# mvrl/RANGE

Hardware: AMD Instinct MI355X
Metric: geo-embeddings/sec (10k-query batch, range_db_large) (higher is better)
Workload: dtype f32

## Files before the change

### range_amd/csrc/engine_ctx.h

```cpp
#pragma once

struct Switches {
    bool allow_keep = true;
    bool enc_split = true;
    bool enc_fused = true;
    bool topks_force_exact = false;
    bool topks_bf16 = true;
    bool topks_fused = true;
    bool small_forward = true;
    bool topk_gemm = true;
    int tg_sample = TG_SAMPLE;
    bool p2_streamk = true;
};

static Switches parse_switches() {
    Switches sw;
    if (const char* e = std::getenv("RANGE_KEEP_LOGITS")) sw.allow_keep = e[0] != '0';
    if (const char* e = std::getenv("RANGE_ENC_SPLIT")) sw.enc_split = e[0] != '0';
    if (const char* e = std::getenv("RANGE_ENC_FUSED")) sw.enc_fused = e[0] != '0';
    if (const char* e = std::getenv("RANGE_TOPKS_FORCE_EXACT")) sw.topks_force_exact = e[0] == '1';
    if (const char* e = std::getenv("RANGE_TOPKS_KEYS")) sw.topks_bf16 = std::strcmp(e, "f32") != 0;
    if (const char* e = std::getenv("RANGE_TOPKS_FUSED")) sw.topks_fused = e[0] != '0';
    if (const char* e = std::getenv("RANGE_SMALL_FORWARD")) sw.small_forward = e[0] != '0';
    if (const char* e = std::getenv("RANGE_TOPK_GEMM")) sw.topk_gemm = e[0] != '0';
    if (const char* e = std::getenv("RANGE_TG_SAMPLE")) sw.tg_sample = std::max(1, std::min(16, std::atoi(e)));
    if (const char* e = std::getenv("RANGE_P2_STREAMK")) sw.p2_streamk = e[0] != '0';
    return sw;
}

struct range_ctx {
    int device = 0;
    int n_cu = 256;
    Switches sw;
    struct Encoder {
        bool has_encoder = false;
        range_encoder_desc desc{};
        EncArgs args{};
        size_t lds_bytes = 0;
        size_t lds_base = 0;
        DevBuf<int32_t> d_slot_base;
        DevBuf<double> d_coefA, d_coefB, d_seedc;
        DevBuf<double> d_wp[ENC_MAX_LAYERS], d_bias[ENC_MAX_LAYERS];
        DevBuf<SHDesc> d_sh_desc;
        DevBuf<double> d_sh_coef;
        DevBuf<int32_t> d_sh_pow;
        DevBuf<double> ws_h1, ws_h1a, ws_h2, ws_e3;
        DevBuf<uint32_t> ws_enc_sync;
    } enc;
    struct Bank {
        bool has_bank = false;
        bool has_values = false;
        int64_t n_rows = 0, n_pad = 0, row_offset = 0;
        DevBuf<float> d_keys, d_values, d_xyz4;
        DevBuf<uint32_t> d_keys_bf16;
        DevBuf<uint32_t> d_keys_f16;
        float tg_key_scale = 0.f;
        float key_norm_max = 1.f;
        float xyz_norm_max = 1.f;
        int pv_mode = RANGE_PV_EXACT;
        DevBuf<uint32_t> d_vplanes;
        int64_t vplanes_groups = 0;
    } bank;
    float tau_sem_set = 0.f, tau_geo_set = 0.f;
    struct Passes {
        DevBuf<double> ws_ehat64;
        DevBuf<float> ws_ehat32, ws_xq, ws_stats;
        int64_t ws_queries = 0;
        DevBuf<float> ws_stats_parts, ws_slabs;
        DevBuf<float> ws_small_o, ws_small_z;
        int last_qtiles = 0, last_splits = 0;
    } pass;
    struct Kept {
        DevBuf<float> ws_logits, ws_rowmax, ws_theta;
        DevBuf<float> ws_stat_parts;
        int64_t kept_B = 0, kept_total = 0;
        int32_t kept_blocks = 0;
        bool warned_no_keep = false;
    } kept;
    struct Topk {
// ... 2 lines not shown
        DevBuf<unsigned long long> ws_cand_keys;
        DevBuf<float> ws_cand_dmax;
        DevBuf<int32_t> ws_exact_count;
        DevBuf<uint32_t> ws_topk_sync;
        uint32_t topk_sync_base[8] = {0, 0, 0, 0, 0, 0, 0, 0};
        DevBuf<float> ws_tg_gmax, ws_tg_theta;
        DevBuf<uint32_t> ws_tg_qfrag;
        DevBuf<float> ws_tg_qscale;
        DevBuf<uint32_t> ws_tg_cnt, ws_tg_ovf;
        DevBuf<uint2> ws_tg_cand;
        DevBuf<uint32_t> ws_read_sink;
    } topk;
    struct Posenc {
        struct Table { std::vector<double> host; DevBuf<double> dev; };
        std::vector<std::unique_ptr<Table>> tables;
    } posenc;
    struct Csp {
        bool has = false;
        int kind = 0, F = 0, act = 0;
        bool skip = false, layn = false;
        int widths[CSP_MAX_LAYERS] = {};
        CspPlan plan;
        DevBuf<float> d_params;
        DevBuf<double> d_freq;
        DevBuf<CspLayerArgs> d_layers;
        int num_classes = 0;
        DevBuf<float> d_head;
        DevBuf<float> ws_feats;
        DevBuf<double> ws_rank;
    } csp;
    struct Checker {
        DevBuf<double> ws_a;
        DevBuf<int64_t> ws_idx;
    } checker;
    struct Neighbors {
        int64_t N = 0;
        int C = 0;
        bool hav = false, has_cells = false;
        DevBuf<NeighborPoint> d_pts;
        DevBuf<int32_t> ws_counts;
        DevBuf<double> ws_redk;
        DevBuf<int64_t> ws_jlast;
    } nb;
    uint32_t* h_async_err = nullptr;
    uint32_t* d_async_err = nullptr;
    bool debug_giveup_next = false;
    struct Host {
        DevBuf<double> ws_out64;
        void* h_stage = nullptr;
        size_t h_stage_bytes = 0;
        hipStream_t copy_stream = nullptr;
        std::unique_ptr<HostCopyPool> pool;
    } host;
    struct Profiling {
        bool on = false;
        std::vector<std::pair<hipEvent_t, hipEvent_t>> pairs[RANGE_PROF_KINDS];
    } prof;
    std::vector<hipEvent_t> ev_pool;
    hipEvent_t get_event() {
        if (!ev_pool.empty()) { hipEvent_t e = ev_pool.back(); ev_pool.pop_back(); return e; }
        hipEvent_t e = nullptr;
        (void)hipEventCreate(&e);
        return e;
    }
    ~range_ctx() {
        if (host.h_stage) (void)hipHostFree(host.h_stage);
        if (h_async_err) (void)hipHostFree(h_async_err);
        if (host.copy_stream) (void)hipStreamDestroy(host.copy_stream);
        for (auto& v : prof.pairs) for (auto& p : v) { (void)hipEventDestroy(p.first); (void)hipEventDestroy(p.second); }
        for (auto e : ev_pool) (void)hipEventDestroy(e);
    }
};

namespace {
struct ProfScope {
    range_ctx* c; int which; hipStream_t s; hipEvent_t a = nullptr, b = nullptr;
    ProfScope(range_ctx* c_, int which_, hipStream_t s_) : c(c_), which(which_), s(s_) {
        if (c->prof.on) { a = c->get_event(); b = c->get_event(); if (a) (void)hipEventRecord(a, s); }
    }
    ~ProfScope() {
        if (a && b) { (void)hipEventRecord(b, s); c->prof.pairs[which].emplace_back(a, b); }
    }
};

constexpr PlanConsts PLAN_CONSTS{QTILE, BLK, VAL_DIM, MAX_TOPK, P1_WG_PER_CU, ENC_QTILE, TOPKS_WL,
                                 TG_QBLOCK, TG_WG_PER_CU, TG_CAP_L};

template <typename... P, typename... A>
int launch(void (*kernel)(P...), dim3 grid, dim3 block, size_t lds, hipStream_t s, const A&... args) {
    if (lds)
        HIP_TRY(hipFuncSetAttribute(reinterpret_cast<const void*>(kernel),
                                    hipFuncAttributeMaxDynamicSharedMemorySize, (int)lds));
    hipLaunchKernelGGL(kernel, grid, block, lds, s, args...);
    HIP_TRY(hipGetLastError());
    return RANGE_OK;
}

template <typename F>
int timed_repeat(range_ctx* c, hipStream_t s, int repeats, float* avg_us, F&& body) {
    hipEvent_t ev0 = nullptr, ev1 = nullptr;
    if (repeats > 1) {
        ev0 = c->get_event();
        ev1 = c->get_event();
        HIP_TRY(hipEventRecord(ev0, s));
    }
    for (int rep = 0; rep < std::max(1, repeats); ++rep)
        if (int rc = body()) return rc;
    if (repeats > 1) {
        HIP_TRY(hipEventRecord(ev1, s));
        HIP_TRY(hipEventSynchronize(ev1));
        float ms = 0.f;
        HIP_TRY(hipEventElapsedTime(&ms, ev0, ev1));
        if (avg_us) *avg_us = ms * 1e3f / (float)repeats;
        c->ev_pool.push_back(ev0);
        c->ev_pool.push_back(ev1);
    }
    return RANGE_OK;
}

}

// ... 15 lines not shown
```

### range_amd/csrc/forward_host.h

```cpp
#pragma once

struct ModelParams { float tau_sem, tau_geo, beta; };

static int model_params(const range_ctx* c, int32_t model, float beta, ModelParams& m) {
    if (model != RANGE_MODEL_RANGE && model != RANGE_MODEL_RANGE_PLUS)
        return fail(RANGE_ERR_INVALID, "unknown model %d", model);
    m.tau_sem = model == RANGE_MODEL_RANGE ? 15.0f : 12.0f;
    m.tau_geo = model == RANGE_MODEL_RANGE ? 0.0f : 40.0f;
    if (c->tau_sem_set > 0.f) m.tau_sem = c->tau_sem_set;
    if (c->tau_geo_set > 0.f && model == RANGE_MODEL_RANGE_PLUS) m.tau_geo = c->tau_geo_set;
    m.beta = model == RANGE_MODEL_RANGE ? 1.0f : beta;
    return RANGE_OK;
}

static int forward_head(const range_ctx* c, const double* lonlat, const double* out, int32_t model, float beta, ModelParams& m) {
    if (!c || !lonlat || !out) return fail(RANGE_ERR_INVALID, "null argument");
    return model_params(c, model, beta, m);
}

static int forward_small(range_ctx* c, int64_t B, const ModelParams& m, double* out, hipStream_t s) {
    SmallArgs a{};
    int rc = softmax_scales(c, B, m.tau_sem, m.tau_geo, RANGE_MAX_TAU, a.k_sem, a.k_geo);
    if (rc) return rc;
    const SmallPlan p = plan_forward_small(c->n_cu, c->bank.n_rows, B, PLAN_CONSTS);
    HIP_TRY(c->pass.ws_small_o.ensure(p.o_floats));
    HIP_TRY(c->pass.ws_small_z.ensure(p.z_floats));
    a.keys = c->bank.d_keys.p;
    a.xyz4 = c->bank.d_xyz4.p;
    a.values = c->bank.d_values.p;
    a.ehat = c->pass.ws_ehat32.p;
    a.xq = c->pass.ws_xq.p;
    a.osum = c->pass.ws_small_o.p;
    a.zsum = c->pass.ws_small_z.p;
    a.B = B;
    a.n_valid = c->bank.n_rows;
    a.n_blocks = p.n_blocks;
    const bool geo = m.tau_geo > 0.f;
    static void (*const small_kernels[2][2])(SmallArgs) = {{attend_small_kernel<true, 2>, attend_small_kernel<true, 1>},
                                                          {attend_small_kernel<false, 2>, attend_small_kernel<false, 1>}};
    {
        ProfScope ps(c, RANGE_PROF_ATTEND, s);
        if (int lrc = launch(small_kernels[!geo][p.nq == 1], dim3((unsigned)p.n_wg), dim3(256), as_lds_bytes(p.nq), s, a)) return lrc;
    }
    rc = launch(small_finalize_kernel, dim3((unsigned)B, 8), dim3(1024), 0, s, c->pass.ws_small_o.p, c->pass.ws_small_z.p,
                p.n_wg, p.qcap, geo ? 1 : 0, geo ? m.beta : 1.0f, c->pass.ws_ehat64.p, out);
    if (rc) return rc;
    c->pass.last_qtiles = 1;
    c->pass.last_splits = p.n_wg;
    return RANGE_OK;
}

static int scan_workspace(range_ctx* c, int64_t B, const ModelParams& m, bool* kept, range_stream_t stream) {
    const int rc = range_scan_stats(c, c->pass.ws_ehat32.p, c->pass.ws_xq.p, B, m.tau_sem, m.tau_geo, c->pass.ws_stats.p, 0,
                                    nullptr, nullptr, 1, stream);
    *kept = c->kept.kept_B == B;
    return rc;
}

static int attend_workspace(range_ctx* c, int64_t p0, int64_t p1, const ModelParams& m, bool kept, SlabMap* map,
                            range_stream_t stream) {
    return attend_impl(c, c->pass.ws_ehat32.p + p0 * 256, c->pass.ws_xq.p + p0 * 4, p1 - p0, m.tau_sem, m.tau_geo, m.beta,
                       c->pass.ws_stats.p + p0 * 4, nullptr, map, kept ? p0 : -1, stream);
}

extern "C" {

int range_forward(range_ctx* c, const double* lonlat, int64_t B, int32_t model, float beta,
                  double* out, range_stream_t stream) {
    ModelParams m;
    if (int rc = forward_head(c, lonlat, out, model, beta, m)) return rc;
    c->pass.ws_queries = 0;
    if (int rc = encode_to_workspace(c, lonlat, B, nullptr, stream)) return rc;
    if (plan_temperatures(m.tau_sem, m.tau_geo, B, c->sw.small_forward).one_pass) {
        c->pass.ws_queries = B;
        ENTER_DEVICE(c);
        return forward_small(c, B, m, out, (hipStream_t)stream);
    }
    bool kept = false;
    SlabMap map{};
    if (int rc = scan_workspace(c, B, m, &kept, stream)) return rc;
    if (int rc = attend_workspace(c, 0, B, m, kept, &map, stream)) return rc;
    c->pass.ws_queries = B;
    ENTER_DEVICE(c);
    HIP_TRY(launch_finalize(c->pass.ws_slabs.p, map, c->pass.ws_ehat64.p, B, 0, B, out, (hipStream_t)stream));
    return RANGE_OK;
}

int range_host_copy(range_ctx* c, void* dst, const void* src, size_t bytes) {
    if (!c || !dst || !src) return fail(RANGE_ERR_INVALID, "null argument");
    if (!c->host.pool) c->host.pool.reset(new HostCopyPool(HostCopyPool::default_threads()));
    c->host.pool->copy(dst, src, bytes);
    return RANGE_OK;
}

int range_forward_host(range_ctx* c, const double* lonlat, int64_t B, int32_t model, float beta,
                       double* out_host, range_stream_t stream) {
    ModelParams m;
    if (int rc0 = forward_head(c, lonlat, out_host, model, beta, m)) return rc0;
    if (B <= 0) return fail(RANGE_ERR_INVALID, "B must be > 0");
    ENTER_DEVICE(c);
    hipStream_t s = (hipStream_t)stream;
    const size_t row_bytes = (size_t)RANGE_OUT_DIM * sizeof(double);
    HIP_TRY(c->host.ws_out64.ensure((size_t)B * RANGE_OUT_DIM));
    if (c->host.h_stage_bytes < (size_t)B * row_bytes) {
        if (c->host.h_stage) (void)hipHostFree(c->host.h_stage);
        c->host.h_stage = nullptr;
        c->host.h_stage_bytes = 0;
        HIP_TRY(hipHostMalloc(&c->host.h_stage, (size_t)B * row_bytes, hipHostMallocDefault));
        c->host.h_stage_bytes = (size_t)B * row_bytes;
    }
    if (!c->host.copy_stream) HIP_TRY(hipStreamCreateWithFlags(&c->host.copy_stream, hipStreamNonBlocking));
    if (!c->host.pool) c->host.pool.reset(new HostCopyPool(HostCopyPool::default_threads()));

    c->pass.ws_queries = 0;
    int rc = encode_to_workspace(c, lonlat, B, nullptr, stream);
    if (rc) return rc;
    c->pass.ws_queries = B;
    if (plan_temperatures(m.tau_sem, m.tau_geo, B, c->sw.small_forward).one_pass) {
        rc = forward_small(c, B, m, c->host.ws_out64.p, s);
        if (rc) return rc;
        HIP_TRY(hipMemcpyAsync(c->host.h_stage, c->host.ws_out64.p, (size_t)B * row_bytes, hipMemcpyDeviceToHost, s));
        HIP_TRY(hipStreamSynchronize(s));
        if (int rc2 = check_async_error(c)) return rc2;
        std::memcpy(out_host, c->host.h_stage, (size_t)B * row_bytes);
        return RANGE_OK;
    }
    bool kept = false;
    rc = scan_workspace(c, B, m, &kept, stream);
    if (rc) return rc;
// ... 56 lines not shown
```

### range_amd/csrc/host_plan.h

```cpp
#pragma once
#include <algorithm>
#include <cmath>
#include <cstddef>
#include <cstdint>
#include <vector>

namespace range_host {

inline int choose_splits(int n_qtiles, int n_blocks, int n_cu, int wg_per_cu, int max_splits,
                         double split_cost = 0.002) {
    const double slots = (double)n_cu * wg_per_cu;
    const int cap = std::max(1, std::min(max_splits, n_blocks / 4));
    const int ns_min = std::min(cap, (int)std::ceil(slots / n_qtiles));
    int best = ns_min;
    double best_score = -1e9;
    for (int ns = ns_min; ns <= cap; ++ns) {
        const double total = (double)n_qtiles * ns;
        const double rounds = std::ceil(total / slots);
        double score = total / (rounds * slots);
        if (rounds < 4) score *= 0.85 + 0.0375 * rounds;
        score -= split_cost * (ns - ns_min);
        if (score > best_score) { best_score = score; best = ns; }
        if (ns - ns_min > 64) break;
    }
// ... 291 lines not shown
    p.n_blocks = (int32_t)((n_rows + K.blk - 1) / K.blk);
    p.n_qtiles = (int32_t)((B + K.qtile - 1) / K.qtile);
    const bool few = B <= 4 * K.qtile;
    p.n_splits = choose_splits(p.n_qtiles, p.n_blocks, n_cu, K.p1_wg_per_cu,
                               topk_scan ? (few ? 256 : 16) : (few ? 2048 : 128));
    if (force_splits > 0) p.n_splits = std::max(1, std::min<int>(force_splits, std::max(1, p.n_blocks / 4)));
    p.grid = p.n_splits * p.n_qtiles;
    p.merge_by_wave = p.n_splits > 32;
    p.part_floats = (size_t)p.n_splits * B * 4;
    p.topk_slots = (B + 15) / 16;
    p.topk_chunks = (int)std::max<int64_t>(1, std::min<int64_t>(
        std::min<int64_t>(64, p.n_blocks / 32 > 0 ? p.n_blocks / 32 : 1),
        ((int64_t)16 * n_cu + p.topk_slots - 1) / p.topk_slots));
    return p;
}

struct KeptStatsPlan {
    int n_qtiles = 0, n_blocks = 0, n_splits = 0;
    int grid = 0;
    bool merge_by_wave = false;
    struct Group { int first, count; };
    std::vector<Group> groups;
    size_t part_floats = 0;
    size_t ws_floats = 0;
};

inline ShiftMode kept_pair_shift(float tau_sem, float tau_geo) { return plan_temperatures(tau_sem, tau_geo, 0, false).shift; }

inline KeptStatsPlan plan_kept_stats(int n_cu, int64_t n_rows, int64_t B, int n_pairs, int force_splits, int max_pairs,
                                     const PlanConsts& K) {
    KeptStatsPlan p;
    const Pass1Plan s = plan_pass1(n_cu, n_rows, B, false, force_splits, K);
    p.n_qtiles = s.n_qtiles;
    p.n_blocks = s.n_blocks;
    p.n_splits = s.n_splits;
    p.grid = s.grid;
    p.merge_by_wave = s.merge_by_wave;
    p.part_floats = s.part_floats;
    for (int first = 0; first < n_pairs; first += max_pairs)
        p.groups.push_back({first, std::min(max_pairs, n_pairs - first)});
    p.ws_floats = p.part_floats * (size_t)std::min(max_pairs, std::max(n_pairs, 0));
    return p;
}

struct Pass2Plan {
    int n_qtiles = 0, n_blocks = 0;
    int n_splits = 0;
    bool streamk = false;
    int sk_cols = 1, sk_groups = 0;
    int grid = 0;
    size_t slab_floats = 0;
};

inline Pass2Plan plan_pass2(int n_cu, int64_t n_rows, int64_t B, bool allow_streamk, const PlanConsts& K) {
    Pass2Plan p;
    p.n_blocks = (int32_t)((n_rows + K.blk - 1) / K.blk);
    p.n_qtiles = (int32_t)((B + K.qtile - 1) / K.qtile);
    p.n_splits = choose_splits(p.n_qtiles, p.n_blocks, n_cu, 1,
                               std::max(32, std::min(512, (n_cu + p.n_qtiles - 1) / p.n_qtiles)),
                               std::max(0.001, 140.0 / (double)n_rows));
    constexpr int P2_STREAMK_ROWS = 50000;
    p.streamk = allow_streamk && n_rows <= P2_STREAMK_ROWS;
    if (p.streamk) {
        constexpr int P2_COL_ROWS = 16384;
        p.sk_cols = (int32_t)std::max<int64_t>(1, std::min<int64_t>((n_rows + P2_COL_ROWS - 1) / P2_COL_ROWS,
                                                                    std::max(1, p.n_blocks / 4)));
        const int64_t Uc = (int64_t)p.n_qtiles * (p.n_blocks / p.sk_cols);
        p.sk_groups = (int32_t)std::max<int64_t>(1, std::min<int64_t>(n_cu, Uc / 4));
        p.slab_floats = (size_t)p.sk_cols * (p.sk_groups + p.n_qtiles) * K.qtile * K.val_dim;
    } else {
        p.slab_floats = (size_t)p.n_splits * B * K.val_dim;
    }
    p.grid = p.streamk ? p.sk_groups : p.n_splits * p.n_qtiles;
    return p;
}

struct TopkPlan {
    int n_groups = 0, n_blocks = 0;
    bool gemm = false;
    int G = 1;
    int n_wg = 0;
    bool fused = false;
    size_t cand_keys = 0, cand_dmax = 0;
    int key_e2 = 0;
    int n_qblocks = 0, n_splits = 0, grid = 0;
    int tile_stride = 1;
};

inline TopkPlan plan_topk(int n_cu, int64_t n_rows, int64_t B, float key_norm_max, bool topk_gemm, bool bf16,
                          bool topks_fused, bool force_exact, int tg_sample, const PlanConsts& K) {
    TopkPlan p;
    p.n_groups = (int)((B + 15) / 16);
    p.n_blocks = (int)((n_rows + K.blk - 1) / K.blk);
    constexpr int NWV = 4;
    p.G = p.n_groups <= 1 ? 1 : 2;
    p.n_wg = std::max(1, std::min(std::min(n_cu, 256), (p.n_blocks + NWV - 1) / NWV));
    p.fused = topks_fused && B <= p.n_wg;
    p.cand_keys = (size_t)p.n_groups * 16 * p.n_wg * K.topks_wl;
    p.cand_dmax = (size_t)p.n_groups * 16 * p.n_wg;
    (void)std::frexp((double)key_norm_max, &p.key_e2);
    const bool tg_bank_ok = key_norm_max > 0.f && std::isfinite(key_norm_max) && std::abs(14 - p.key_e2) <= 100;
    p.gemm = topk_gemm && bf16 && B > 256 && p.n_blocks >= 64 && !force_exact && B <= 60000 && tg_bank_ok;
    if (p.gemm) {
        p.n_qblocks = (int32_t)((B + K.tg_qblock - 1) / K.tg_qblock);
        p.n_splits = std::max(4, std::min(std::min(K.tg_wg_per_cu * n_cu / p.n_qblocks, p.n_blocks / 8), 64));
        p.grid = p.n_qblocks * p.n_splits;
        p.tile_stride = std::max(1, std::min(tg_sample, p.n_blocks / p.n_splits / 4));
    }
    return p;
}

struct SmallPlan {
    int n_blocks = 0, n_wg = 0;
    int nq = 1, qcap = 16;
    size_t o_floats = 0, z_floats = 0;
};

inline SmallPlan plan_forward_small(int n_cu, int64_t n_rows, int64_t B, const PlanConsts& K) {
    SmallPlan p;
    p.n_blocks = (int)((n_rows + K.blk - 1) / K.blk);
    p.n_wg = std::max(1, std::min(n_cu, p.n_blocks));
    p.nq = B > 16 ? 2 : 1;
    p.qcap = 16 * p.nq;
    p.o_floats = (size_t)p.n_wg * 2 * p.qcap * K.val_dim;
    p.z_floats = (size_t)p.n_wg * p.qcap * 2;
    return p;
// ... 535 lines not shown
```

### range_amd/csrc/range_hip.hip

```cpp
#include <hip/hip_runtime.h>

#include <algorithm>
#include <cmath>
#include <cstdarg>
#include <cstdio>
#include <cstdlib>
#include <cstring>
#include <memory>
#include <string>
#include <vector>

#include "../../include/range_hip.h"
#include "host_common.h"
#include "host_copy.h"
#include "host_plan.h"
#include "scan_common.h"
#include "topk_lists.h"
#include "pass1.h"
#include "pass1_sharp.h"
#include "pass1_kept.h"
#include "pass2.h"
#include "topk_stream.h"
#include "topk_gemm.h"
#include "attend_bf16x3.h"
#include "attend_small.h"
#include "encoder_kernel.h"
#include "posenc_kernel.h"
#include "csp_kernel.h"
#include "csp_head_kernel.h"
#include "csp_rank_kernel.h"
#include "checker_kernel.h"
#include "neighbor_kernel.h"

using namespace range_hip;
using namespace range_host;

#include "engine_ctx.h"
#include "encoder_host.h"
#include "bank_host.h"
#include "scan_host.h"
#include "topk_host.h"
#include "forward_host.h"
#include "posenc_host.h"
#include "csp_host.h"
#include "checker_host.h"
#include "neighbor_host.h"

extern "C" {

int range_abi_version(void) { return RANGE_ABI_VERSION; }
const char* range_last_error(void) { return g_err.c_str(); }
#ifndef RANGE_BUILD_FLAGS
#define RANGE_BUILD_FLAGS ""
#endif
const char* range_build_flags(void) { return RANGE_BUILD_FLAGS; }
#ifndef RANGE_SRC_SHA256
#define RANGE_SRC_SHA256 "unknown"
#endif
static const char g_src_stamp[] = "RANGE_SRC_SHA256=" RANGE_SRC_SHA256;
const char* range_source_sha256(void) { return g_src_stamp + 17; }

int range_create(int device, range_ctx** out) {
    if (!out) return fail(RANGE_ERR_INVALID, "out is null");
    *out = nullptr;
    int count = 0;
    HIP_TRY(hipGetDeviceCount(&count));
    if (device < 0 || device >= count)
        return fail(RANGE_ERR_INVALID, "device %d out of range (%d visible)", device, count);
    hipDeviceProp_t prop;
    HIP_TRY(hipGetDeviceProperties(&prop, device));
    if (std::strncmp(prop.gcnArchName, "gfx950", 6) != 0)
        return fail(RANGE_ERR_INVALID, "device %d is %s; this library is built for gfx950 only",
                    device, prop.gcnArchName);
    range_ctx* c = new (std::nothrow) range_ctx();
// ... 90 lines not shown
```

### range_amd/csrc/scan_common.h

```cpp
#pragma once
#include "engine_prims.h"
#include "host_plan.h"

namespace range_hip {

struct ScanArgs {
    const float* keys;
    const float* xyz4;
    const float* values;
    const float* ehat;
    const float* xq;
    const float* stats;
    float* out;
    float* cand_val;
    int32_t* cand_idx;
    int64_t B;
    int64_t n_valid;
    int32_t n_blocks;
    int32_t n_qtiles;
    int32_t n_splits;
    float k_sem;
    float k_geo;
    float beta;
    unsigned long long* diag;
    float* logits;
    int32_t qt_offset;
    float* rowmax;
    int32_t sk_groups;
    int32_t sk_cols;
};

struct SlabMap {
    int32_t n_parts;
    int32_t sk_groups;
    int32_t n_blocks;
    int32_t n_qtiles;
    int32_t sk_cols;
};
using range_host::sk_owner;
using range_host::sk_start, range_host::sk_col_begin;
__device__ __forceinline__ void slab_parts(const SlabMap& m, int64_t B, int64_t q, int c, int64_t& first4, int64_t& stride4, int& count) {
    if (m.sk_groups == 0) {
        first4 = q * (VAL_DIM / 4);
        stride4 = B * (VAL_DIM / 4);
        count = m.n_parts;
        return;
    }
    const int64_t cb = sk_col_begin(c + 1, m.n_blocks, m.sk_cols) - sk_col_begin(c, m.n_blocks, m.sk_cols);
    const int64_t qt = q / QTILE, U = (int64_t)m.n_qtiles * cb;
    const int64_t w0 = sk_owner(qt * cb, U, m.sk_groups), w1 = sk_owner((qt + 1) * cb - 1, U, m.sk_groups);
    first4 = (((int64_t)c * (m.sk_groups + m.n_qtiles) + w0 + qt) * QTILE + (q - qt * QTILE)) * (VAL_DIM / 4);
    stride4 = (int64_t)QTILE * (VAL_DIM / 4);
    count = (int)(w1 - w0) + 1;
}
__device__ __forceinline__ int slab_cols(const SlabMap& m) { return m.sk_groups == 0 ? 1 : m.sk_cols; }

__device__ __forceinline__ int64_t logit_tile(int64_t qtile, int32_t n_blocks, int block, int wave) {
    return ((qtile * n_blocks + block) * 4 + wave) * 256;
}

__device__ __forceinline__ void decode_block(const ScanArgs& a, int& split, int& qt) {
    const int total = a.n_splits * a.n_qtiles;
    const int b = blockIdx.x;
    const int x = b & 7, j = b >> 3;
    const int q = total >> 3, r = total & 7;
    const int item = x * q + (x < r ? x : r) + j;
    split = item / a.n_qtiles;
    qt = item - split * a.n_qtiles;
}

struct QFrag {
    f32x4 q[16];
    float xq;
};

__device__ __forceinline__ void load_qfrag(QFrag& f, const float* ehat, const float* xq, int64_t B,
                                           int64_t q, int g) {
    const int64_t qq = q < B ? q : B - 1;
    const f32x4* row = reinterpret_cast<const f32x4*>(ehat + qq * KEY_DIM);
#pragma unroll
    for (int s = 0; s < 16; ++s) f.q[s] = row[4 * s + g];
    f.xq = xq[qq * 4 + g];
}

__device__ __forceinline__ void pin_qfrag(QFrag& f) {
#pragma unroll
    for (int s = 0; s < 16; ++s) asm volatile("" : "+v"(f.q[s]));
    asm volatile("" : "+v"(f.xq));
}


struct QKAcc {
    f32x4 a0, g;
    __device__ __forceinline__ float sem(int r) const { return a0[r]; }
    __device__ __forceinline__ void fence() {
        asm volatile("s_nop 15" : "+v"(a0), "+v"(g));
    }
};

struct KAddr {
    uint32_t b[4];
    uint32_t x;
    __device__ __forceinline__ void init(int lane) {
        const int g = lane >> 4;
        const int R = pi_row(lane & 15);
#pragma unroll
        for (int bb = 0; bb < 4; ++bb)
            b[bb] = (uint32_t)(R * (KEY_DIM * 4) + 64 * (bb ^ (R >> 2)) + 16 * (g ^ (R & 3)));
        x = (uint32_t)((R * 4 + g) * 4);
    }
};

struct KFirst { f32x4 k0, k1; float xa; };

template <bool GEO>
__device__ __forceinline__ KFirst qk_first_reads(const char* kt, const char* xt, const KAddr& ka_) {
    KFirst r;
    r.k0 = *reinterpret_cast<const f32x4*>(kt + ka_.b[0]);
    r.k1 = *reinterpret_cast<const f32x4*>(kt + ka_.b[1]);
    r.xa = GEO ? *reinterpret_cast<const float*>(xt + ka_.x) : 0.f;
    return r;
}
// ... 45 lines not shown
```

### range_amd/csrc/scan_host.h

```cpp
#pragma once

static_assert(MAX_TAU_CONSTANT == RANGE_MAX_TAU && MAX_TAU_SHARP == RANGE_MAX_TAU_SHARP, "host_plan.h and range_hip.h disagree");

static int softmax_scales(range_ctx* c, int64_t B, float tau_sem, float tau_geo, float max_tau, float& k_sem, float& k_geo) {
    if (!c->bank.has_bank) return fail(RANGE_ERR_STATE, "bank not set (range_set_bank)");
    if (!c->bank.has_values)
        return fail(RANGE_ERR_STATE, "keys-only bank (range_set_keys): only range_topk_stream runs on it");
    if (B <= 0) return fail(RANGE_ERR_INVALID, "B must be > 0");
    if (!plan_temperatures(tau_sem, tau_geo, B, false).valid)
        return fail(RANGE_ERR_INVALID, "temperatures must be finite, > 0 and at most %g (tau_sem %g, tau_geo %g; tau_geo <= 0: "
                    "no geographic head): beyond that the softmax is an argmax to float32 precision",
                    (double)RANGE_MAX_TAU_SHARP, (double)tau_sem, (double)tau_geo);
    if (!(c->bank.key_norm_max <= 1.001f))
        return fail(RANGE_ERR_INVALID, "bank keys are not L2-normalised or not finite (largest row norm %.4f): the softmax of "
                    "range_scan_stats / range_attend needs unit keys, as range/range.py:85-89 prepares them "
                    "(range_topk_stream accepts any norm)", (double)c->bank.key_norm_max);
    if (tau_geo > 0.f && !(c->bank.xyz_norm_max <= 1.001f))
        return fail(RANGE_ERR_INVALID, "bank locations are not unit vectors or not finite (largest row norm %.4f): the geographic "
                    "softmax needs them as range/utils/utils.py:11-16 computes them", (double)c->bank.xyz_norm_max);
    if (tau_sem > max_tau || tau_geo > max_tau)
        return fail(RANGE_ERR_INVALID, "internal: temperatures above %g reached a constant-shift kernel", (double)max_tau);
    const double LOG2E = 1.4426950408889634;
    k_sem = (float)(tau_sem * LOG2E);
    k_geo = tau_geo > 0.f ? (float)(tau_geo * LOG2E) : 0.f;
    return RANGE_OK;
}

static int fill_scan_args(range_ctx* c, ScanArgs& a, const float* ehat32, const float* xq, int64_t B,
                          float tau_sem, float tau_geo) {
    if (int rc = softmax_scales(c, B, tau_sem, tau_geo, RANGE_MAX_TAU_SHARP, a.k_sem, a.k_geo)) return rc;
    a.keys = c->bank.d_keys.p;
    a.xyz4 = c->bank.d_xyz4.p;
    a.values = c->bank.d_values.p;
    a.ehat = ehat32;
    a.xq = xq;
    a.B = B;
    a.n_valid = c->bank.n_rows;
    a.beta = 1.f;
    a.sk_cols = 1;
    return RANGE_OK;
}

static int launch_merge_stats(bool by_wave, const float* parts, int32_t n_parts, int64_t B, float* out, hipStream_t s) {
    const int per_wg = by_wave ? 4 : 256;
    return launch(by_wave ? merge_stats_wave_kernel : merge_stats_kernel, dim3((unsigned)((B + per_wg - 1) / per_wg)), dim3(256),
                  0, s, parts, n_parts, B, out);
}

static hipError_t launch_finalize(const float* slabs, const SlabMap& map, const double* ehat64, int64_t B, int64_t q0,
                                  int64_t nq, double* out, hipStream_t s) {
    const int64_t n = nq * 320;
    hipLaunchKernelGGL(finalize_kernel, dim3((unsigned)((n + 255) / 256)), dim3(256), 0, s, slabs, map, ehat64, B, q0, nq, out);
    return hipGetLastError();
}

static int scan_stats_impl(range_ctx* c, const float* ehat32, const float* xq32, int64_t B, float tau_sem,
                           float tau_geo, float* stats, int topk, float* topk_val, int64_t* topk_idx,
                           int32_t keep_logits, int64_t first_query, int64_t total_queries, int32_t force_splits,
                           range_stream_t stream) {
    if (!c || !ehat32 || !xq32 || !stats) return fail(RANGE_ERR_INVALID, "null argument");
    if (topk < 0 || topk > MAX_TOPK) return fail(RANGE_ERR_INVALID, "topk must be in [0,%d]", MAX_TOPK);
    if (topk > 0 && (!topk_val || !topk_idx)) return fail(RANGE_ERR_INVALID, "topk outputs null");
    if (first_query < 0 || first_query % QTILE != 0)
        return fail(RANGE_ERR_INVALID, "first_query must be a non-negative multiple of %d", QTILE);
    if (B > 0 && first_query + B > total_queries)
        return fail(RANGE_ERR_INVALID, "queries [%lld, %lld) exceed the scan's %lld", (long long)first_query,
                    (long long)(first_query + B), (long long)total_queries);
    if (force_splits < 0) return fail(RANGE_ERR_INVALID, "n_splits must be >= 0");
    ENTER_DEVICE(c);
    ScanArgs a{};
    hipStream_t s = (hipStream_t)stream;
    const bool extends = first_query > 0 && c->kept.kept_B == first_query && c->kept.kept_total == total_queries;
    if (first_query > 0 && !extends) keep_logits = 0;
    if (!extends) c->kept.kept_B = 0;
    bool write_logits = c->sw.allow_keep && (topk > 0 ? B > 0 : keep_logits != 0);
    const int64_t n_qtiles = (total_queries + QTILE - 1) / QTILE, n_blocks = (c->bank.n_rows + BLK - 1) / BLK;
    const size_t need = (size_t)n_qtiles * n_blocks * 1024;
    if (write_logits && extends) {
        if (need > c->kept.ws_logits.n || c->kept.kept_blocks != n_blocks) { write_logits = false; c->kept.kept_B = 0; }
    } else if (write_logits && need > c->kept.ws_logits.n) {
        size_t free_b = 0, total_b = 0;
        HIP_TRY(hipMemGetInfo(&free_b, &total_b));
        if (need * sizeof(float) <= free_b / 2) {
            HIP_TRY(c->kept.ws_logits.ensure(need));
        } else {
            write_logits = false;
            if (!c->kept.warned_no_keep) {
                c->kept.warned_no_keep = true;
                std::fprintf(stderr, "librange_hip: the logits of %lld queries x %lld bank rows (%.1f GB) do not fit in "
                             "half of the free device memory (%.1f GB free): not kept, pass 2 recomputes them\n",
                             (long long)B, (long long)c->bank.n_rows, need * 4e-9, free_b * 1e-9);
            }
        }
    }
    const bool topk_from_kept = topk > 0 && write_logits;
    const bool topk_scan = topk > 0 && !topk_from_kept;
    int rc = fill_scan_args(c, a, ehat32, xq32, B, tau_sem, tau_geo);
    if (rc) return rc;
    const TempRoute route = plan_temperatures(tau_sem, tau_geo, B, c->sw.small_forward);
    if (topk_scan && !route.topk_scan_ok)
        return fail(RANGE_ERR_INVALID, "range_scan_stats(topk > 0) at a temperature above %g needs to keep its logits (this "
                    "context cannot: RANGE_KEEP_LOGITS=0 or not enough free memory): take the top-k from range_topk_stream",
                    (double)RANGE_MAX_TAU);
    const Pass1Plan p = plan_pass1(c->n_cu, c->bank.n_rows, B, topk_scan, force_splits, PLAN_CONSTS);
    a.n_blocks = p.n_blocks;
    a.n_qtiles = p.n_qtiles;
    a.n_splits = p.n_splits;
    if (write_logits) a.logits = c->kept.ws_logits.p;
    a.qt_offset = (int32_t)(first_query / QTILE);
    if (topk_from_kept) {
        HIP_TRY(c->kept.ws_rowmax.ensure(p.part_floats));
        HIP_TRY(c->kept.ws_theta.ensure((size_t)B));
        a.rowmax = c->kept.ws_rowmax.p;
    }
    HIP_TRY(c->pass.ws_stats_parts.ensure(p.part_floats));
    a.out = c->pass.ws_stats_parts.p;
    if (topk_scan) {
        HIP_TRY(c->topk.ws_cand_val.ensure(p.part_floats * MAX_TOPK));
        HIP_TRY(c->topk.ws_cand_idx.ensure(p.part_floats * MAX_TOPK));
        a.cand_val = c->topk.ws_cand_val.p;
        a.cand_idx = c->topk.ws_cand_idx.p;
    }
    const bool geo = tau_geo > 0.f;
    static void (*const scan_kernels[2][2])(ScanArgs) = {{scan_stats_kernel<true, true>, scan_stats_kernel<true, false>},
                                                        {scan_stats_kernel<false, true>, scan_stats_kernel<false, false>}};
    static void (*const sharp_kernels[2])(ScanArgs) = {sharp_scan_stats_kernel<true>, sharp_scan_stats_kernel<false>};
    {
        ProfScope ps(c, RANGE_PROF_SCAN_STATS, s);
        void (*const kernel)(ScanArgs) = route.shift == SHIFT_RUNNING_MAX ? sharp_kernels[!geo] : scan_kernels[!geo][!topk_scan];
        if (int lrc = launch(kernel, dim3((unsigned)p.grid), dim3(256), SCAN_LDS_BYTES, s, a)) return lrc;
    }
    if (a.logits && keep_logits) {
        c->kept.kept_B = first_query + B;
        c->kept.kept_total = total_queries;
        c->kept.kept_blocks = a.n_blocks;
    }
    rc = launch_merge_stats(p.merge_by_wave, c->pass.ws_stats_parts.p, a.n_splits, B, stats, s);
    if (rc) return rc;
    int n_parts = a.n_splits, per_part = 4 * MAX_TOPK;
    if (topk_from_kept) {
        const int n_chunks = p.topk_chunks;
        HIP_TRY(c->topk.ws_cand_val.ensure((size_t)n_chunks * B * MAX_TOPK));
        HIP_TRY(c->topk.ws_cand_idx.ensure((size_t)n_chunks * B * MAX_TOPK));
        rc = launch(topk_threshold_kernel, dim3((unsigned)((B + 3) / 4)), dim3(256), 0, s,
                    c->kept.ws_rowmax.p, a.n_splits, B, c->kept.ws_theta.p);
        if (rc) return rc;
        rc = launch(topk_from_logits_kernel, dim3((unsigned)((p.topk_slots + 3) / 4), (unsigned)n_chunks),
                    dim3(256), 0, s, c->kept.ws_logits.p, a.n_blocks, B, c->bank.n_rows, n_chunks,
                    c->kept.ws_theta.p, c->topk.ws_cand_val.p, c->topk.ws_cand_idx.p);
        if (rc) return rc;
        n_parts = n_chunks;
        per_part = MAX_TOPK;
    }
    if (topk <= 0) return RANGE_OK;
    return launch(merge_topk_wave_kernel, dim3((unsigned)((B + 3) / 4)), dim3(256), 0, s, c->topk.ws_cand_val.p,
                  c->topk.ws_cand_idx.p, n_parts, B, per_part, topk, c->bank.row_offset, topk_val, topk_idx);
}

static int attend_impl(range_ctx* c, const float* ehat32, const float* xq32, int64_t B, float tau_sem,
                       float tau_geo, float beta, const float* stats_global, float* partial,
                       SlabMap* map_out, int64_t kept_first, range_stream_t stream,
                       unsigned long long* diag_dev = nullptr, int64_t diag_capacity = 0) {
    if (!c || (!ehat32 && kept_first < 0) || !xq32 || !stats_global)
        return fail(RANGE_ERR_INVALID, "null argument");
    if (kept_first >= 0) {
        if (c->kept.kept_B <= 0) return fail(RANGE_ERR_STATE, "no kept logits (range_scan_stats with keep_logits)");
        if (kept_first % QTILE != 0) return fail(RANGE_ERR_INVALID, "first kept query must be a multiple of %d", QTILE);
        if (kept_first + B > c->kept.kept_B)
            return fail(RANGE_ERR_INVALID, "queries [%lld, %lld) exceed the %lld kept", (long long)kept_first,
                        (long long)(kept_first + B), (long long)c->kept.kept_B);
    }
    if (!diag_dev && !(beta >= 0.f && beta <= 1.f)) return fail(RANGE_ERR_INVALID, "beta must be in [0,1]");
    ENTER_DEVICE(c);
    ScanArgs a{};
    int rc = fill_scan_args(c, a, ehat32, xq32, B, tau_sem, tau_geo);
    if (rc) return rc;
    hipStream_t s = (hipStream_t)stream;
    const bool geo = tau_geo > 0.f;
    const bool bf16x3 = kept_first >= 0 && c->bank.pv_mode == RANGE_PV_BF16X3;
    if (bf16x3 && plan_temperatures(tau_sem, tau_geo, B, false).shift == SHIFT_RUNNING_MAX)
        return fail(RANGE_ERR_INVALID, "pv mode bf16x3 is not supported at temperatures above %g", (double)RANGE_MAX_TAU);
    const Pass2Plan p = plan_pass2(c->n_cu, c->bank.n_rows, B, c->sw.p2_streamk && !bf16x3 && !diag_dev, PLAN_CONSTS);
    a.n_blocks = p.n_blocks;
    a.n_qtiles = p.n_qtiles;
    a.n_splits = p.n_splits;
    a.sk_cols = p.sk_cols;
    a.sk_groups = p.sk_groups;
    c->pass.last_qtiles = p.n_qtiles;
    c->pass.last_splits = p.streamk ? p.sk_groups : p.n_splits;
    if (diag_dev) {
        if (!geo) return fail(RANGE_ERR_INVALID, "diagnostic build exists for the geo variant only");
        if ((int64_t)p.grid * 4 * 16 > diag_capacity) return fail(RANGE_ERR_INVALID, "diag buffer too small");
    }
    HIP_TRY(c->pass.ws_slabs.ensure(p.slab_floats));
    const SlabMap map{a.n_splits, a.sk_groups, a.n_blocks, a.n_qtiles, a.sk_cols};
    a.out = c->pass.ws_slabs.p;
    a.stats = stats_global;
    a.beta = geo ? beta : 1.f;
    const dim3 grid((unsigned)p.grid), block(256);
    static void (*const bf16x3_kernels[2])(ScanArgs, const char*, int32_t) = {attend_bf16x3_kernel<true>,
                                                                             attend_bf16x3_kernel<false>};
    static void (*const stored_kernels[2])(ScanArgs) = {attend_stored_kernel<true>, attend_stored_kernel<false>};
    static void (*const recompute_kernels[2])(ScanArgs) = {attend_kernel<true>, attend_kernel<false>};
    if (diag_dev) {
        a.diag = diag_dev;
        return launch(attend_kernel<true, true>, grid, block, ATTEND_LDS_BYTES, s, a);
    }
    if (kept_first >= 0) {
        if (a.n_blocks != c->kept.kept_blocks) return fail(RANGE_ERR_STATE, "bank changed since the logits were kept");
        a.logits = c->kept.ws_logits.p;
        a.qt_offset = (int32_t)(kept_first / QTILE);
        ProfScope ps(c, RANGE_PROF_ATTEND, s);
        if (bf16x3) {
            const int32_t n_groups = (a.n_blocks + 1) / 2;
            if (c->bank.vplanes_groups != n_groups) return fail(RANGE_ERR_STATE, "bf16 planes of the values are missing");
            const char* planes = reinterpret_cast<const char*>(c->bank.d_vplanes.p);
            rc = launch(bf16x3_kernels[!geo], grid, block, PVB2_LDS_BYTES, s, a, planes, n_groups);
        } else {
            rc = launch(stored_kernels[!geo], grid, block, ATTEND_STORED_LDS_BYTES, s, a);
        }
    } else {
        ProfScope ps(c, RANGE_PROF_ATTEND, s);
        rc = launch(recompute_kernels[!geo], grid, block, ATTEND_LDS_BYTES, s, a);
    }
    if (rc) return rc;
    if (map_out) *map_out = map;
    if (partial) {
        const int64_t total4 = B * (VAL_DIM / 4);
        return launch(reduce_parts_kernel, dim3((unsigned)((total4 + 255) / 256)), dim3(256), 0, s,
                      c->pass.ws_slabs.p, map, B, partial);
    }
    return RANGE_OK;
}

extern "C" {
// ... 150 lines not shown
```

Before: 524,400.

## Overlap chunked pass 1 on an aux stream with pass 2 attention

Splits the forward batch into query-tile chunks sized to fill the CUs. Pass 1 for later chunks runs on an auxiliary stream, using a new persistent, lower-LDS scan kernel that can sit beside pass 2, while pass 2 and finalize for earlier chunks run on the main stream with event dependencies. The goal is to hide pass 1 latency and the tail idle time between the two passes. The cost is more host launches, a forced split count for pass 2, and a new kernel that does not use the regular pass 1 path. Chunked mode only applies with constant shift, exact PV and a non-streamk pass 2.

After: 530,700, median of 6. +1.2%, better.

```diff
diff --git a/range_amd/csrc/engine_ctx.h b/range_amd/csrc/engine_ctx.h
--- a/range_amd/csrc/engine_ctx.h
+++ b/range_amd/csrc/engine_ctx.h
@@ -11,6 +11,7 @@
     bool topk_gemm = true;
     int tg_sample = TG_SAMPLE;
     bool p2_streamk = true;
+    int fwd_overlap = -1;
 };
 
 static Switches parse_switches() {
@@ -25,6 +26,7 @@
     if (const char* e = std::getenv("RANGE_TOPK_GEMM")) sw.topk_gemm = e[0] != '0';
     if (const char* e = std::getenv("RANGE_TG_SAMPLE")) sw.tg_sample = std::max(1, std::min(16, std::atoi(e)));
     if (const char* e = std::getenv("RANGE_P2_STREAMK")) sw.p2_streamk = e[0] != '0';
+    if (const char* e = std::getenv("RANGE_FWD_OVERLAP")) sw.fwd_overlap = std::max(0, std::atoi(e));
     return sw;
 }
 
@@ -133,6 +135,10 @@
         hipStream_t copy_stream = nullptr;
         std::unique_ptr<HostCopyPool> pool;
     } host;
+    struct Overlap {
+        hipStream_t aux_stream = nullptr;
+        std::vector<hipEvent_t> events;
+    } ovl;
     struct Profiling {
         bool on = false;
         std::vector<std::pair<hipEvent_t, hipEvent_t>> pairs[RANGE_PROF_KINDS];
@@ -148,6 +154,8 @@
         if (host.h_stage) (void)hipHostFree(host.h_stage);
         if (h_async_err) (void)hipHostFree(h_async_err);
         if (host.copy_stream) (void)hipStreamDestroy(host.copy_stream);
+        if (ovl.aux_stream) (void)hipStreamDestroy(ovl.aux_stream);
+        for (auto e : ovl.events) (void)hipEventDestroy(e);
         for (auto& v : prof.pairs) for (auto& p : v) { (void)hipEventDestroy(p.first); (void)hipEventDestroy(p.second); }
         for (auto e : ev_pool) (void)hipEventDestroy(e);
     }
diff --git a/range_amd/csrc/forward_host.h b/range_amd/csrc/forward_host.h
--- a/range_amd/csrc/forward_host.h
+++ b/range_amd/csrc/forward_host.h
@@ -63,6 +63,64 @@
                        c->pass.ws_stats.p + p0 * 4, nullptr, map, kept ? p0 : -1, stream);
 }
 
+static int forward_chunked(range_ctx* c, int64_t B, const ModelParams& m, const FwdChunkPlan& plan, double* out,
+                           range_stream_t stream, bool* chunked) {
+    *chunked = false;
+    ENTER_DEVICE(c);
+    hipStream_t s = (hipStream_t)stream;
+    const size_t n_chunks = plan.tiles.size();
+    if (!c->ovl.aux_stream) {
+        HIP_TRY(hipStreamCreateWithFlags(&c->ovl.aux_stream, hipStreamNonBlocking));
+    }
+    while (c->ovl.events.size() < n_chunks) {
+        hipEvent_t e = nullptr;
+        HIP_TRY(hipEventCreateWithFlags(&e, hipEventDisableTiming));
+        c->ovl.events.push_back(e);
+    }
+    int64_t most_tiles = 0;
+    for (int t : plan.tiles) most_tiles = std::max<int64_t>(most_tiles, t);
+    HIP_TRY(c->pass.ws_stats_parts.ensure((size_t)plan.p1_splits * B * 4));
+    HIP_TRY(c->pass.ws_slabs.ensure((size_t)plan.p2_splits * std::min<int64_t>(B, most_tiles * QTILE) * VAL_DIM));
+    const float* ehat = c->pass.ws_ehat32.p;
+    const float* xq = c->pass.ws_xq.p;
+    float* stats = c->pass.ws_stats.p;
+    std::vector<int64_t> cuts{0};
+    for (int t : plan.tiles) cuts.push_back(std::min<int64_t>(B, cuts.back() + (int64_t)t * QTILE));
+    if (int rc = scan_stats_impl(c, ehat, xq, cuts[1], m.tau_sem, m.tau_geo, stats, 0, nullptr, nullptr, 1, 0, B,
+                                 plan.p1_splits, stream))
+        return rc;
+    if (c->kept.kept_B != cuts[1]) return RANGE_OK;
+    *chunked = true;
+    HIP_TRY(hipEventRecord(c->ovl.events[0], s));
+    HIP_TRY(hipStreamWaitEvent(c->ovl.aux_stream, c->ovl.events[0], 0));
+    size_t recorded = 0;
+    auto joined = [&](int rc) {
+        (void)hipStreamWaitEvent(s, c->ovl.events[recorded], 0);
+        return rc;
+    };
+    for (size_t i = 1; i < n_chunks; ++i) {
+        const int64_t q0 = cuts[i], nq = cuts[i + 1] - q0;
+        if (int rc = scan_stats_impl(c, ehat + q0 * KEY_DIM, xq + q0 * 4, nq, m.tau_sem, m.tau_geo, stats + q0 * 4, 0, nullptr, nullptr,
+                                     1, q0, B, plan.p1_splits, (range_stream_t)c->ovl.aux_stream, true,
+                                     (size_t)plan.p1_splits * q0 * 4))
+            return joined(rc);
+        HIP_TRY(hipEventRecord(c->ovl.events[i], c->ovl.aux_stream));
+        recorded = i;
+    }
+    for (size_t i = 0; i < n_chunks; ++i) {
+        const int64_t q0 = cuts[i], nq = cuts[i + 1] - q0;
+        if (i > 0) HIP_TRY(hipStreamWaitEvent(s, c->ovl.events[i], 0));
+        SlabMap map{};
+        if (int rc = attend_impl(c, ehat + q0 * KEY_DIM, xq + q0 * 4, nq, m.tau_sem, m.tau_geo, m.beta, stats + q0 * 4, nullptr, &map, q0,
+                                 stream, nullptr, 0, plan.p2_splits))
+            return joined(rc);
+        HIP_TRY(launch_finalize(c->pass.ws_slabs.p, map, c->pass.ws_ehat64.p + q0 * KEY_DIM, nq, 0, nq, out + q0 * RANGE_OUT_DIM, s));
+    }
+    c->pass.last_qtiles = (int)((B + QTILE - 1) / QTILE);
+    c->pass.last_splits = plan.p2_splits;
+    return RANGE_OK;
+}
+
 extern "C" {
 
 int range_forward(range_ctx* c, const double* lonlat, int64_t B, int32_t model, float beta,
@@ -75,6 +133,20 @@
         c->pass.ws_queries = B;
         ENTER_DEVICE(c);
         return forward_small(c, B, m, out, (hipStream_t)stream);
+    }
+    if (c->sw.allow_keep && c->bank.pv_mode == RANGE_PV_EXACT && c->bank.has_bank &&
+        plan_temperatures(m.tau_sem, m.tau_geo, B, false).shift == SHIFT_CONSTANT) {
+        const FwdChunkPlan plan = plan_forward_chunks(c->n_cu, plan_pass1(c->n_cu, c->bank.n_rows, B, false, 0, PLAN_CONSTS),
+                                                      plan_pass2(c->n_cu, c->bank.n_rows, B, c->sw.p2_streamk, PLAN_CONSTS),
+                                                      c->sw.fwd_overlap);
+        if (plan.tiles.size() >= 2) {
+            bool chunked = false;
+            if (int rc = forward_chunked(c, B, m, plan, out, stream, &chunked)) return rc;
+            if (chunked) {
+                c->pass.ws_queries = B;
+                return RANGE_OK;
+            }
+        }
     }
     bool kept = false;
     SlabMap map{};
diff --git a/range_amd/csrc/host_plan.h b/range_amd/csrc/host_plan.h
--- a/range_amd/csrc/host_plan.h
+++ b/range_amd/csrc/host_plan.h
@@ -367,13 +367,15 @@
     size_t slab_floats = 0;
 };
 
-inline Pass2Plan plan_pass2(int n_cu, int64_t n_rows, int64_t B, bool allow_streamk, const PlanConsts& K) {
+inline Pass2Plan plan_pass2(int n_cu, int64_t n_rows, int64_t B, bool allow_streamk, const PlanConsts& K,
+                            int force_splits = 0) {
     Pass2Plan p;
     p.n_blocks = (int32_t)((n_rows + K.blk - 1) / K.blk);
     p.n_qtiles = (int32_t)((B + K.qtile - 1) / K.qtile);
     p.n_splits = choose_splits(p.n_qtiles, p.n_blocks, n_cu, 1,
                                std::max(32, std::min(512, (n_cu + p.n_qtiles - 1) / p.n_qtiles)),
                                std::max(0.001, 140.0 / (double)n_rows));
+    if (force_splits > 0) p.n_splits = std::max(1, std::min<int>(force_splits, std::max(1, p.n_blocks / 4)));
     constexpr int P2_STREAMK_ROWS = 50000;
     p.streamk = allow_streamk && n_rows <= P2_STREAMK_ROWS;
     if (p.streamk) {
@@ -387,6 +389,51 @@
         p.slab_floats = (size_t)p.n_splits * B * K.val_dim;
     }
     p.grid = p.streamk ? p.sk_groups : p.n_splits * p.n_qtiles;
+    return p;
+}
+
+struct FwdChunkPlan {
+    std::vector<int> tiles;
+    int p1_splits = 0, p2_splits = 0;
+};
+
+constexpr int FWD_CHUNK_FILL_PCT = 98;
+inline FwdChunkPlan plan_forward_chunks(int n_cu, const Pass1Plan& p1, const Pass2Plan& p2, int overlap) {
+    FwdChunkPlan p;
+    p.p1_splits = p1.n_splits;
+    p.p2_splits = p2.n_splits;
+    const int T = p2.n_qtiles, ns = p2.n_splits;
+    if (overlap == 0 || p2.streamk || T < 2 || ns < 1 || n_cu < 1) return p;
+    if (overlap > 0) {
+        for (int t0 = 0; t0 < T && overlap < T; t0 += overlap) p.tiles.push_back(std::min(overlap, T - t0));
+        return p;
+    }
+    const int64_t R = ((int64_t)T * ns + n_cu - 1) / n_cu;
+    for (int64_t C = std::min<int64_t>(R, T); C >= 2; --C) {
+        std::vector<int> lo((size_t)C), hi((size_t)C);
+        int64_t sum_lo = 0, sum_hi = 0;
+        bool ok = true;
+        for (int64_t i = 0; i < C && ok; ++i) {
+            const int64_t r = R / C + (i >= C - R % C ? 1 : 0);
+            const int64_t most = r * n_cu / ns;
+            const int64_t fill = (FWD_CHUNK_FILL_PCT * r * n_cu + 100 * (int64_t)ns - 1) / (100 * (int64_t)ns);
+            const int64_t least = std::max<int64_t>(std::max<int64_t>(fill, (r - 1) * n_cu / ns + 1), 1);
+            ok = least <= most;
+            lo[(size_t)i] = (int)least;
+            hi[(size_t)i] = (int)most;
+            sum_lo += least;
+            sum_hi += most;
+        }
+        if (!ok || sum_lo > T || sum_hi < T) continue;
+        p.tiles = hi;
+        int64_t excess = sum_hi - T;
+        for (size_t i = 0; i < p.tiles.size() && excess > 0; ++i) {
+            const int64_t d = std::min<int64_t>(excess, hi[i] - lo[i]);
+            p.tiles[i] -= (int)d;
+            excess -= d;
+        }
+        return p;
+    }
     return p;
 }
 
diff --git a/range_amd/csrc/pass1_beside.h b/range_amd/csrc/pass1_beside.h
--- /dev/null
+++ b/range_amd/csrc/pass1_beside.h
@@ -0,0 +1,140 @@
+#pragma once
+#include <type_traits>
+
+#include "pass1.h"
+#include "pass2.h"
+
+namespace range_hip {
+
+constexpr uint32_t BESIDE_HALF_BYTES = BLK * (KEY_DIM / 2) * 4;
+constexpr int BESIDE_LDS_BYTES = 2 * BESIDE_HALF_BYTES + 2 * 64 * 4;
+static_assert(ATTEND_STORED_LDS_BYTES + BESIDE_LDS_BYTES <= 160 * 1024, "pass 1 must fit beside pass 2 in a CU's LDS");
+
+struct KAddrHalf {
+    uint32_t b[4];
+    uint32_t x;
+    __device__ __forceinline__ void init(int lane) {
+        const int g = lane >> 4;
+        const int R = pi_row(lane & 15);
+#pragma unroll
+        for (int bb = 0; bb < 4; ++bb)
+            b[bb] = (uint32_t)(R * (KEY_DIM * 2) + 64 * (bb ^ (R >> 2)) + 16 * (g ^ (R & 3)));
+        x = (uint32_t)((R * 4 + g) * 4);
+    }
+};
+
+__device__ __forceinline__ void issue_k_half(const float* keys, int64_t row0, int half, uint32_t slot_lds, int wave,
+                                             const uint32_t (&voff)[2]) {
+#pragma unroll
+    for (int d = 0; d < 2; ++d) {
+        const int R0 = 4 * wave + 2 * d;
+        dma_b128(keys + (row0 + R0) * KEY_DIM, voff[d] + (uint32_t)half * (KEY_DIM * 2), slot_lds + R0 * (KEY_DIM * 2));
+    }
+}
+
+template <int H>
+__device__ __forceinline__ void qk_mfma_half(const char* kh, const KAddrHalf& ka_, const QFrag& f, f32x4& a0) {
+    f32x4 kn = *reinterpret_cast<const f32x4*>(kh + ka_.b[0]);
+    f32x4 kn2 = *reinterpret_cast<const f32x4*>(kh + ka_.b[1]);
+#pragma unroll
+    for (int s = 0; s < 8; ++s) {
+        const f32x4 ka = kn;
+        kn = kn2;
+        if (s < 6) kn2 = *reinterpret_cast<const f32x4*>(kh + ka_.b[(s + 2) & 3] + 256 * ((s + 2) >> 2));
+        const int S = 8 * H + s;
+        if (S == 0) mfma_v_first(a0, ka.x, f.q[S].x);
+        else mfma_v(a0, ka.x, f.q[S].x);
+        mfma_v(a0, ka.y, f.q[S].y);
+        mfma_v(a0, ka.z, f.q[S].z);
+        mfma_v(a0, ka.w, f.q[S].w);
+    }
+}
+
+template <bool GEO>
+__global__ __launch_bounds__(256) __attribute__((amdgpu_waves_per_eu(3))) void scan_stats_beside_kernel(ScanArgs a) {
+    extern __shared__ __attribute__((aligned(16))) char smem[];
+    const uint32_t lds0 = (uint32_t)(uintptr_t)RANGE_LPTR(smem);
+    const uint32_t xring_lds = lds0 + 2 * BESIDE_HALF_BYTES;
+
+    const int lane = threadIdx.x & 63;
+    const int wave = __builtin_amdgcn_readfirstlane(threadIdx.x >> 6);
+    const int g = lane >> 4;
+    KAddrHalf kaddr;
+    kaddr.init(lane);
+    uint32_t voff[2];
+#pragma unroll
+    for (int d = 0; d < 2; ++d) {
+        const int R = 4 * wave + 2 * d + (lane >> 5);
+        voff[d] = (uint32_t)((lane >> 5) * (KEY_DIM * 4) + (((lane & 31) ^ R) << 4));
+    }
+    const float nm1 = -a.k_sem, nm2 = -a.k_geo;
+    const int total = a.n_splits * a.n_qtiles;
+
+    for (int vb = blockIdx.x; vb < total; vb += gridDim.x) {
+        int split, qt;
+        decode_item(a, vb, split, qt);
+        const int b0 = part_begin(split, a.n_blocks, a.n_splits);
+        const int nb = part_begin(split + 1, a.n_blocks, a.n_splits) - b0;
+        const int64_t q = (int64_t)qt * QTILE + wave * 16 + (lane & 15);
+
+        QFrag f;
+        load_qfrag(f, a.ehat, a.xq, a.B, q, g);
+        pin_qfrag(f);
+        float l1 = 0.f, l2 = 0.f;
+
+        if (nb > 0) {
+            issue_k_half(a.keys, (int64_t)b0 * BLK, 0, lds0, wave, voff);
+            dma_b32(a.xyz4 + (int64_t)b0 * BLK * 4, (uint32_t)(lane << 2), xring_lds);
+        }
+        for (int t = 0; t < nb; ++t) {
+            const int64_t row0 = (int64_t)(b0 + t) * BLK;
+            QKAcc c;
+            RANGE_WAIT_BARRIER(0);
+            issue_k_half(a.keys, row0, 1, lds0 + BESIDE_HALF_BYTES, wave, voff);
+            const float xa = GEO ? *reinterpret_cast<const float*>(smem + 2 * BESIDE_HALF_BYTES + (t & 1) * 256 + kaddr.x) : 0.f;
+            qk_mfma_half<0>(smem, kaddr, f, c.a0);
+            RANGE_WAIT_BARRIER(0);
+            if (t + 1 < nb) {
+                issue_k_half(a.keys, row0 + BLK, 0, lds0, wave, voff);
+                dma_b32(a.xyz4 + (row0 + BLK) * 4, (uint32_t)(lane << 2), xring_lds + ((t + 1) & 1) * 256);
+            }
+            qk_mfma_half<1>(smem + BESIDE_HALF_BYTES, kaddr, f, c.a0);
+            if (GEO) mfma_v_first(c.g, xa, f.xq);
+            else c.g = f32x4{0.f, 0.f, 0.f, 0.f};
+            c.fence();
+            const f32x4 ss = {c.sem(0), c.sem(1), c.sem(2), c.sem(3)};
+            const f32x4 sg = c.g;
+            if (a.logits)
+                __builtin_nontemporal_store(ss, reinterpret_cast<f32x4*>(a.logits + logit_tile((int64_t)qt + a.qt_offset, a.n_blocks, b0 + t, wave) + 4 * lane));
+            const int n_here = (int)(a.n_valid - row0 < BLK ? a.n_valid - row0 : BLK);
+            auto tile_stats = [&](auto masked_tag) __attribute__((always_inline)) {
+                constexpr bool MASKED = decltype(masked_tag)::value;
+#pragma unroll
+                for (int r = 0; r < 4; ++r) {
+                    const bool ok = !MASKED || pi_row(4 * g + r) < n_here;
+                    const float p1 = __builtin_amdgcn_exp2f(fmaf(ss[r], a.k_sem, nm1));
+                    l1 += ok ? p1 : 0.f;
+                    if (GEO) {
+                        const float p2 = __builtin_amdgcn_exp2f(fmaf(sg[r], a.k_geo, nm2));
+                        l2 += ok ? p2 : 0.f;
+                    }
+                }
+            };
+            if (n_here == BLK) tile_stats(std::false_type{});
+            else tile_stats(std::true_type{});
+        }
+#pragma unroll
+        for (int off = 16; off <= 32; off <<= 1) {
+            l1 += __shfl_xor(l1, off);
+            if (GEO) l2 += __shfl_xor(l2, off);
+        }
+        float m2 = a.k_geo;
+        if (!GEO) { m2 = NEG_BIG; l2 = 0.f; }
+        if (q < a.B && g == 0) {
+            f32x4 o = {a.k_sem, l1, m2, l2};
+            *reinterpret_cast<f32x4*>(a.out + ((int64_t)split * a.B + q) * 4) = o;
+        }
+    }
+}
+
+}
diff --git a/range_amd/csrc/range_hip.hip b/range_amd/csrc/range_hip.hip
--- a/range_amd/csrc/range_hip.hip
+++ b/range_amd/csrc/range_hip.hip
@@ -20,6 +20,7 @@
 #include "pass1_sharp.h"
 #include "pass1_kept.h"
 #include "pass2.h"
+#include "pass1_beside.h"
 #include "topk_stream.h"
 #include "topk_gemm.h"
 #include "attend_bf16x3.h"
diff --git a/range_amd/csrc/scan_common.h b/range_amd/csrc/scan_common.h
--- a/range_amd/csrc/scan_common.h
+++ b/range_amd/csrc/scan_common.h
@@ -59,15 +59,15 @@
     return ((qtile * n_blocks + block) * 4 + wave) * 256;
 }
 
-__device__ __forceinline__ void decode_block(const ScanArgs& a, int& split, int& qt) {
+__device__ __forceinline__ void decode_item(const ScanArgs& a, int b, int& split, int& qt) {
     const int total = a.n_splits * a.n_qtiles;
-    const int b = blockIdx.x;
     const int x = b & 7, j = b >> 3;
     const int q = total >> 3, r = total & 7;
     const int item = x * q + (x < r ? x : r) + j;
     split = item / a.n_qtiles;
     qt = item - split * a.n_qtiles;
 }
+__device__ __forceinline__ void decode_block(const ScanArgs& a, int& split, int& qt) { decode_item(a, (int)blockIdx.x, split, qt); }
 
 struct QFrag {
     f32x4 q[16];
diff --git a/range_amd/csrc/scan_host.h b/range_amd/csrc/scan_host.h
--- a/range_amd/csrc/scan_host.h
+++ b/range_amd/csrc/scan_host.h
@@ -57,7 +57,7 @@
 static int scan_stats_impl(range_ctx* c, const float* ehat32, const float* xq32, int64_t B, float tau_sem,
                            float tau_geo, float* stats, int topk, float* topk_val, int64_t* topk_idx,
                            int32_t keep_logits, int64_t first_query, int64_t total_queries, int32_t force_splits,
-                           range_stream_t stream) {
+                           range_stream_t stream, bool beside = false, size_t parts_offset = 0) {
     if (!c || !ehat32 || !xq32 || !stats) return fail(RANGE_ERR_INVALID, "null argument");
     if (topk < 0 || topk > MAX_TOPK) return fail(RANGE_ERR_INVALID, "topk must be in [0,%d]", MAX_TOPK);
     if (topk > 0 && (!topk_val || !topk_idx)) return fail(RANGE_ERR_INVALID, "topk outputs null");
@@ -113,8 +113,8 @@
         HIP_TRY(c->kept.ws_theta.ensure((size_t)B));
         a.rowmax = c->kept.ws_rowmax.p;
     }
-    HIP_TRY(c->pass.ws_stats_parts.ensure(p.part_floats));
-    a.out = c->pass.ws_stats_parts.p;
+    HIP_TRY(c->pass.ws_stats_parts.ensure(parts_offset + p.part_floats));
+    a.out = c->pass.ws_stats_parts.p + parts_offset;
     if (topk_scan) {
         HIP_TRY(c->topk.ws_cand_val.ensure(p.part_floats * MAX_TOPK));
         HIP_TRY(c->topk.ws_cand_idx.ensure(p.part_floats * MAX_TOPK));
@@ -125,17 +125,24 @@
     static void (*const scan_kernels[2][2])(ScanArgs) = {{scan_stats_kernel<true, true>, scan_stats_kernel<true, false>},
                                                         {scan_stats_kernel<false, true>, scan_stats_kernel<false, false>}};
     static void (*const sharp_kernels[2])(ScanArgs) = {sharp_scan_stats_kernel<true>, sharp_scan_stats_kernel<false>};
+    static void (*const beside_kernels[2])(ScanArgs) = {scan_stats_beside_kernel<true>, scan_stats_beside_kernel<false>};
+    if (beside && (topk > 0 || route.shift == SHIFT_RUNNING_MAX))
+        return fail(RANGE_ERR_INVALID, "internal: pass 1 beside pass 2 has the constant shift and no top-k");
     {
         ProfScope ps(c, RANGE_PROF_SCAN_STATS, s);
-        void (*const kernel)(ScanArgs) = route.shift == SHIFT_RUNNING_MAX ? sharp_kernels[!geo] : scan_kernels[!geo][!topk_scan];
-        if (int lrc = launch(kernel, dim3((unsigned)p.grid), dim3(256), SCAN_LDS_BYTES, s, a)) return lrc;
+        if (beside) {
+            if (int lrc = launch(beside_kernels[!geo], dim3((unsigned)std::min(c->n_cu, p.grid)), dim3(256), BESIDE_LDS_BYTES, s, a)) return lrc;
+        } else {
+            void (*const kernel)(ScanArgs) = route.shift == SHIFT_RUNNING_MAX ? sharp_kernels[!geo] : scan_kernels[!geo][!topk_scan];
+            if (int lrc = launch(kernel, dim3((unsigned)p.grid), dim3(256), SCAN_LDS_BYTES, s, a)) return lrc;
+        }
     }
     if (a.logits && keep_logits) {
         c->kept.kept_B = first_query + B;
         c->kept.kept_total = total_queries;
         c->kept.kept_blocks = a.n_blocks;
     }
-    rc = launch_merge_stats(p.merge_by_wave, c->pass.ws_stats_parts.p, a.n_splits, B, stats, s);
+    rc = launch_merge_stats(p.merge_by_wave, a.out, a.n_splits, B, stats, s);
     if (rc) return rc;
     int n_parts = a.n_splits, per_part = 4 * MAX_TOPK;
     if (topk_from_kept) {
@@ -160,7 +167,7 @@
 static int attend_impl(range_ctx* c, const float* ehat32, const float* xq32, int64_t B, float tau_sem,
                        float tau_geo, float beta, const float* stats_global, float* partial,
                        SlabMap* map_out, int64_t kept_first, range_stream_t stream,
-                       unsigned long long* diag_dev = nullptr, int64_t diag_capacity = 0) {
+                       unsigned long long* diag_dev = nullptr, int64_t diag_capacity = 0, int32_t force_splits = 0) {
     if (!c || (!ehat32 && kept_first < 0) || !xq32 || !stats_global)
         return fail(RANGE_ERR_INVALID, "null argument");
     if (kept_first >= 0) {
@@ -180,7 +187,7 @@
     const bool bf16x3 = kept_first >= 0 && c->bank.pv_mode == RANGE_PV_BF16X3;
     if (bf16x3 && plan_temperatures(tau_sem, tau_geo, B, false).shift == SHIFT_RUNNING_MAX)
         return fail(RANGE_ERR_INVALID, "pv mode bf16x3 is not supported at temperatures above %g", (double)RANGE_MAX_TAU);
-    const Pass2Plan p = plan_pass2(c->n_cu, c->bank.n_rows, B, c->sw.p2_streamk && !bf16x3 && !diag_dev, PLAN_CONSTS);
+    const Pass2Plan p = plan_pass2(c->n_cu, c->bank.n_rows, B, c->sw.p2_streamk && !bf16x3 && !diag_dev, PLAN_CONSTS, force_splits);
     a.n_blocks = p.n_blocks;
     a.n_qtiles = p.n_qtiles;
     a.n_splits = p.n_splits;
```
